# Enhex/RGK

Hardware: AMD Instinct MI355X
Metric: Mpaths/s, Sponza 1920x1080x256spp (path-tracing hot path) (higher is better)
Workload: dtype f32; 1 GPU; sponza-1080p 1920x1080x256spp depth 2 russian 0.74, strong scaling; geometry=proxy, triangles=64536, sampler=halton-cp, textures=handed over as u8; 0 of 0 float textures stored as bytes + value table, tiles=2040, parallelism=tiles round-robin over 1 GPU(s) + one RCCL reduce per round

## Files before the change

rgk_amd/csrc/rgk_host.cpp:

```cpp
#include <hip/hip_runtime.h>

#include <algorithm>
#include <array>
#include <atomic>
#include <cmath>
#include <cstdio>
#include <cstdlib>
#include <cstring>
#include <string>
#include <vector>

#include "../../include/rgk.h"
#include "device_types.h"
#include "rgk_commit.h"
#include "rgk_kernels.h"
#include "rgk_build.h"
#include "rgk_adapt.h"

namespace {

#define HIPCHK(x)                                                                                     \
    do {                                                                                              \
        hipError_t e_ = (x);                                                                          \
        if (e_ != hipSuccess)                                                                         \
// ... 23 lines not shown
            (void)hipDeviceSynchronize();
        }
        return 0;
    }
    int upload(const T* src, size_t count) {
        int rc = alloc(count);
        if (rc) return rc;
        if (count) {
            hipError_t e = hipMemcpy(p, src, count * sizeof(T), hipMemcpyHostToDevice);
            if (e != hipSuccess) return fail(RGK_ERR_DEVICE, "hipMemcpy H2D: %s", hipGetErrorString(e));
        }
        return 0;
    }
    void release() { if (p) (void)hipFree(p); p = nullptr; n = 0; }
};

}

struct RgkTuning {
    bool entry_points = true;
    bool entry_cap = true;
    bool light_entry = true;
    bool const_light = true;
    int sample_group = -1;
    size_t batch_paths = 0;
    double workspace_gb = 0;
    int beam = 1;
    bool debug_bvh = false, debug_util = false;
    bool time_post = false;
};

enum PostSlot : uint32_t { POST_AOV = 0, POST_DENOISE = 1, POST_DENOISE_VARIANCE = 2, POST_NOISE = 3, POST_FOLD = 4, POST_SLOTS = 5 };
constexpr uint32_t RGK_SCENE_MAGIC = 0x53474b52u;
struct rgk_scene {
    uint32_t magic = RGK_SCENE_MAGIC;
    int device = 0;
    RgkTuning tune;
    hipStream_t stream = nullptr;
    rgk_scene_info info{};
    DevScene dev{};
    RgkTraceCfg tcfg{32, 32, nullptr};
    DevBuf<int> ovf;
    DevBuf<QNode> nodes;
    DevBuf<TriIsect> tris;
    DevBuf<TriShade> tri_shade;
    DevBuf<DevMaterial> materials;
    DevBuf<float4> texels;
    DevBuf<uint32_t> texels8;
    DevBuf<float> luts;
    DevBuf<DevPointLight> pointlights;
    DevPointLight h_light0{};
    DevBuf<DevArealLight> areal;
    DevBuf<DevArealTri> areal_tris;
    DevBuf<float4> ltc;
    DevBuf<DevScene> self;
    DevBuf<uint32_t> generic;
    DevBuf<TexRef> texrefs;
    DevBuf<uint32_t> d_idx;
    DevBuf<float4> leaf_pb;
    std::vector<uint32_t> h_idx, h_tri_mat, h_areal_off, h_areal_tris;
    std::vector<rgk_material> h_mats;
    std::vector<float> h_normals;
    uint32_t n_vertices = 0, n_triangles = 0, n_refs = 0, n_nodes = 0;
    uint32_t n_textures = 0, n_materials = 0;
    DevBuf<DevHaltonDim> hdims;
    DevBuf<uint16_t> hperm;
    size_t batch = 0;
    DevBuf<float4> rayA[2], rayB[2], hit, thr, tot, shA, shB, shC, pixsum, light;
    DevBuf<float4> lstart, lv;
    DevBuf<uint32_t> hitlist;
    DevBuf<uint32_t> lvmask, connlist;
    DevBuf<float4> conn, jobs, rads;
    uint32_t batch_reverse = 0;
    DevBuf<float> htab;
    DevBuf<float2> nearfar;
    DevBuf<uint32_t> counters, pix_xy, pix_seed, tile_buf;
    DevBuf<int> entry;
    DevBuf<float> entry_cap;
    size_t entry_capped = 0;
    DevBuf<int> lentry;
    DevBuf<uint32_t> trange;
    DevBuf<float4> lbox;
    size_t lentry_done = 0;
    uint64_t entry_key = 0;
    size_t entry_n = 0;
    DevBuf<unsigned long long> stats;
    DevBuf<float> scratch_f;
    DevBuf<uint32_t> scratch_u;
    DevBuf<float4> dn_col[2], dn_guide;
    DevBuf<rgk_noise_tile> nz_tiles;
    DevBuf<uint32_t> fold_buf;
// ... 52 lines not shown
template <typename T>
int down(T* dst, const DevBuf<T>& b, size_t count) {
    if (hipMemcpy(dst, b.p, count * sizeof(T), hipMemcpyDeviceToHost) != hipSuccess) return fail(RGK_ERR_DEVICE, "hipMemcpy D2H failed");
    return 0;
}

int scene_event(rgk_scene* s, size_t i, hipEvent_t& e) {
    while (s->events.size() <= i) { hipEvent_t n; HIPCHK(hipEventCreate(&n)); s->events.push_back(n); }
    e = s->events[i];
    return 0;
}

int check_frame_size(uint32_t xres, uint32_t yres) {
    if (xres == 0 || yres == 0 || xres > 65535 || yres > 65535) return fail(RGK_ERR_INVALID, "resolution out of range");
    return RGK_OK;
}

int read_stats(const rgk_scene* s, unsigned long long (&h)[8]) { return down(h, s->stats, 8); }

RgkTuning read_tuning() {
    auto off = [](const char* name) { const char* e = std::getenv(name); return e && e[0] == '0'; };
    RgkTuning t;
    t.entry_points = !off("RGK_ENTRY_POINTS"); t.entry_cap = !off("RGK_ENTRY_CAP"); t.light_entry = !off("RGK_LIGHT_ENTRY");
    t.const_light = !off("RGK_CONST_LIGHT");
    if (const char* e = std::getenv("RGK_SAMPLE_GROUP")) t.sample_group = std::min(6, std::max(0, std::atoi(e)));
    if (const char* e = std::getenv("RGK_BATCH_PATHS")) t.batch_paths = std::max<size_t>(1024, strtoull(e, nullptr, 10));
    if (const char* e = std::getenv("RGK_WORKSPACE_GB")) t.workspace_gb = atof(e);
    if (const char* e = std::getenv("RGK_BEAM")) t.beam = std::min(2, std::max(0, std::atoi(e)));
    t.debug_bvh = std::getenv("RGK_DEBUG_BVH") != nullptr; t.debug_util = std::getenv("RGK_DEBUG_UTIL") != nullptr;
    return t;
}

void invalidate_frame_lists(rgk_scene* s) { s->entry_key = 0; s->entry_n = 0; s->entry_capped = 0; s->lentry_done = 0; }

void set_bounds(rgk_scene* s, const float mn[3], const float mx[3], float eps) {
    DevScene& ds = s->dev;
    ds.epsilon = eps;
    s->info.epsilon = eps;
    for (int a = 0; a < 3; a++) {
        ds.bb_min[a] = mn[a] - eps; ds.bb_max[a] = mx[a] + eps;
        s->info.bbox_min[a] = ds.bb_min[a]; s->info.bbox_max[a] = ds.bb_max[a];
    }
}

struct AccelInfo {
    uint32_t n_nodes = 0, n_refs = 0, max_depth = 0, max_stack = 0;
    bool on_device = false;
// ... 203 lines not shown
int rgk_scene_get_info(const rgk_scene* s, rgk_scene_info* out) {
    if (!s || !out) return fail(RGK_ERR_INVALID, "null argument");
    *out = s->info;
    return RGK_OK;
}

int rgk_scene_get_progress(const rgk_scene* s, rgk_progress* out) {
    if (!s || !out) return fail(RGK_ERR_INVALID, "null argument");
    out->stage = s->h_stage ? *(volatile const uint32_t*)s->h_stage : 0u; out->stages = s->prog_stages.load(); out->rounds = s->prog_rounds.load(); out->busy = s->prog_busy.load();
    out->round_pixels = s->prog_pixels.load(); out->round_paths = s->prog_paths.load();
    if (out->stage > out->stages) out->stage = out->stages;
    return RGK_OK;
}

int rgk_scene_set_tuning(rgk_scene* s, const char* key, double value) {
    if (!s || !key) return fail(RGK_ERR_INVALID, "null argument");
    if (s->prog_busy.load()) return fail(RGK_ERR_INVALID, "rgk_scene_set_tuning while a round is in flight on this scene");
    RgkTuning& t = s->tune;
    const std::string k(key);
    if (k == "entry_points") t.entry_points = value != 0;
    else if (k == "entry_cap") t.entry_cap = value != 0;
    else if (k == "light_entry") t.light_entry = value != 0;
    else if (k == "const_light") t.const_light = value != 0;
    else if (k == "sample_group") t.sample_group = value < 0 ? -1 : (int)std::min(6.0, value);
    else if (k == "batch_paths") t.batch_paths = value <= 0 ? 0 : std::max<size_t>(1024, (size_t)value);
    else if (k == "workspace_gb") t.workspace_gb = value <= 0 ? 0.0 : value;
    else if (k == "beam") t.beam = (int)std::min(2.0, std::max(0.0, value));
    else if (k == "time_post") { t.time_post = value != 0; return RGK_OK; }
    else return fail(RGK_ERR_INVALID, "unknown tuning key '%s'", key);
    invalidate_frame_lists(s);
    return RGK_OK;
}

int rgk_generate_task_list(uint32_t tile_size, uint32_t xres, uint32_t yres, float mid_x, float mid_y, uint32_t seedstart,
                           uint32_t seedcount_base, rgk_tile* tiles, uint32_t* n_tiles) {
    if (!n_tiles || tile_size == 0) return fail(RGK_ERR_INVALID, "bad argument");
    struct T { rgk_tile t; float d; };
    std::vector<T> v;
    for (uint32_t yp = 0; yp < yres; yp += tile_size)
        for (uint32_t xp = 0; xp < xres; xp += tile_size) {
            T t;
            t.t.x0 = xp; t.t.x1 = std::min(xres, xp + tile_size);
            t.t.y0 = yp; t.t.y1 = std::min(yres, yp + tile_size);
            t.t.seed = 0;
            float mx = (t.t.x0 + t.t.x1) / 2.0f, my = (t.t.y0 + t.t.y1) / 2.0f;
            float dx = mid_x - mx, dy = mid_y - my;
// ... 222 lines not shown
    if ((need_cap || need_light) && (rc = kl.run(RGK_K_OTHER, [&] { rgk_launch_group_trange(st, pp, s->hit.p, s->trange.p); }))) return rc;
    if (need_cap) {
        if ((rc = kl.run(RGK_K_OTHER, [&] { rgk_launch_entry_points(st, s->dev, cam, pp.xres, pp.yres, s->pix_xy.p, P, groups.first, groups.count(), s->trange.p, s->entry.p, s->entry_cap.p); })))
            return rc;
        s->entry_capped = end;
    }
    if (!light_entry) return 0;
    pp.lentry = s->lentry.p; pp.lbox = s->lbox.p;
    if (!need_light) return 0;
    if ((rc = kl.run(RGK_K_OTHER, [&] { rgk_launch_light_entry_points(st, s->dev, cam, pp, P, s->trange.p, s->lentry.p, s->lbox.p); }))) return rc;
    s->lentry_done = end;
    if (s->tune.debug_bvh) {
        const size_t g0 = groups.first, g1 = groups.last;
        std::vector<int> he((g1 - g0) * RGK_ENTRY_K);
        HIPCHK(hipStreamSynchronize(st));
        HIPCHK(hipMemcpy(he.data(), s->lentry.p + g0 * RGK_ENTRY_K, he.size() * sizeof(int), hipMemcpyDeviceToHost));
        size_t below = 0, total_e = 0;
        for (size_t g = 0; g < g1 - g0; g++) { if (he[g * RGK_ENTRY_K] != 0) below++; for (int k = 0; k < RGK_ENTRY_K; k++) total_e += he[g * RGK_ENTRY_K + k] != 0x7fffffff; }
        std::fprintf(stderr, "[rgk] light-side entry nodes: %zu of %zu pixel groups start below the root, %.2f entries per group\n", below, g1 - g0, (double)total_e / (double)(g1 - g0));
    }
    return 0;
}

int queue_pass(rgk_scene* s, KernelLog& kl, const DevCamera& cam, PassParams& pp, size_t P, bool light_entry, bool const_light, float* d_accum_rgb,
               uint32_t* d_accum_count, uint32_t stage) {
    hipStream_t st = s->stream;
    const RgkTraceCfg& tc = s->tcfg;
    const bool count_stats = kl.count_stats, cap_entries = s->entry.p != nullptr && s->tune.entry_cap;
    const bool track = pp.depth > 12;
    const uint32_t R = pp.reverse, n0 = pp.npix * pp.ns;
    pp.gshift = rgk_plan_gshift(s->tune.sample_group, RGK_SAMPLE_GROUP_DEFAULT, pp.ns);
    pp.beam = rgk_beam_wanted(s->tune.beam, cap_entries && (size_t)pp.j0 + pp.npix <= s->entry_capped) ? 1u : 0u;
    float4* const rayA[2] = {s->rayA[0].p, s->rayA[1].p};
    float4* const rayB[2] = {s->rayB[0].p, s->rayB[1].p};
    float4 *const hit = s->hit.p, *const thr = s->thr.p, *const tot = s->tot.p, *const shA = s->shA.p, *const shB = s->shB.p, *const shC = s->shC.p;
    uint32_t* const cn = s->counters.p;
    uint32_t* const cl = cn + RGK_CNT_TOTAL;
    int rc;
    if (R > 0) {
        if ((rc = kl.run(RGK_K_OTHER, [&] { rgk_launch_init_counters(st, cl, 0u); })) ||
            (rc = kl.run(RGK_K_LIGHT_SHADE, [&] { rgk_launch_raygen_light(st, s->dev, cam, pp, rayA[0], rayB[0], thr, cl); })))
            return rc;
        for (uint32_t k = 0; k < R; k++) {
            const int q = k & 1;
            if ((rc = kl.run(RGK_K_LIGHT_TRACE, [&] { rgk_launch_trace_closest(st, s->dev, tc, count_stats, rayA[q], rayB[q], nullptr, hit, {n0, cl + RGK_CNT_QUEUE + k, cl + RGK_CNT_FETCH_T + k}, s->stats.p); })) ||
                (rc = kl.run(RGK_K_LIGHT_SHADE, [&] { rgk_launch_list_hits(st, hit, cl + RGK_CNT_QUEUE + k, s->hitlist.p, cl + RGK_CNT_HITS + k, n0); })) ||
                (rc = kl.run(RGK_K_LIGHT_SHADE, [&] { rgk_launch_shade_light(st, s->dev, cam, pp, k, rayA[q], rayB[q], hit, thr, rayA[q ^ 1], rayB[q ^ 1], shA, shB, shC, cl, n0); })) ||
                (rc = kl.run(RGK_K_LIGHT_SPLAT, [&] { rgk_launch_trace_shadow(st, s->dev, tc, count_stats, shA, shB, shC, nullptr, nullptr, RGK_SHADOW_SPLAT, d_accum_rgb,
                                                                              {n0, cl + RGK_CNT_SHADOW + k, cl + RGK_CNT_FETCH_S + k}, s->stats.p); })))
                return rc;
        }
    }
    if ((rc = kl.run(RGK_K_OTHER, [&] { rgk_launch_init_counters(st, cn, n0); }))) return rc;
    uint32_t ub = n0;
    for (uint32_t b = 0; b < pp.depth && ub > 0; b++) {
        const int q = b & 1;
        const RgkWalk wq = {ub, cn + RGK_CNT_QUEUE + b, cn + RGK_CNT_FETCH_T + b}, ws = {ub, cn + RGK_CNT_SHADOW + b, cn + RGK_CNT_FETCH_S + b};
        if (b == 0)
            rc = kl.run(RGK_K_TRACE_CAMERA, [&] { rgk_launch_trace_camera(st, s->dev, cam, pp, tc, count_stats, hit, wq, s->stats.p); });
        else
            rc = kl.run(RGK_K_TRACE_CLOSEST, [&] { rgk_launch_trace_closest(st, s->dev, tc, count_stats, rayA[q], rayB[q], nullptr, hit, wq, s->stats.p); });
        if (rc || (b == 0 && (rc = queue_first_hit_lists(s, kl, cam, pp, (uint32_t)P, cap_entries, light_entry)))) return rc;
        if ((rc = kl.run(b == 0 ? RGK_K_SHADE_FIRST : RGK_K_SHADE, [&] { rgk_launch_shade(st, s->dev, cam, pp, b, rayA[q], rayB[q], hit, thr, tot, rayA[q ^ 1], rayB[q ^ 1], shA, shB, shC, cn, ub, R > 0, const_light); })) ||
            (R > 0 && (rc = kl.run(RGK_K_CONNECT, [&] { rgk_launch_connect(st, s->dev, pp, b, s->jobs.p, s->rads.p, cn, ub); }))))
            return rc;
        const bool first = b == 0 && light_entry, rec32 = const_light && rgk_const_light_records();
        rc = kl.run(first ? RGK_K_SHADOW_FIRST : RGK_K_SHADOW, [&] {
            if (rec32 && first) rgk_launch_trace_shadow_first_cl(st, s->dev, pp, tc, count_stats, shA, shB, tot, ws, s->stats.p);
            else if (rec32) rgk_launch_trace_shadow_cl(st, s->dev, tc, count_stats, shA, shB, tot, ws, s->stats.p);
            else if (first) rgk_launch_trace_shadow_first(st, s->dev, pp, tc, count_stats, shA, shB, shC, tot, ws, s->stats.p);
            else rgk_launch_trace_shadow(st, s->dev, tc, count_stats, shA, shB, shC, tot, nullptr, RGK_SHADOW_ADD, nullptr, ws, s->stats.p);
        });
        if (rc || (R > 0 && (rc = kl.run(RGK_K_SHADOW_JOBS, [&] { rgk_launch_trace_shadow_jobs(st, s->dev, pp, tc, count_stats, s->jobs.p, s->rads.p, tot, {ub, cn + RGK_CNT_CONN + b, cn + RGK_CNT_FETCH_J + b}, s->stats.p); }))))
            return rc;
        rgk_launch_stage_mark(st, s->h_stage, stage + b + 1);
        if (track && b >= 3 && (b & 1) && b + 1 < pp.depth && (rc = queue_len(s, cn + RGK_CNT_QUEUE + b + 1, ub))) return rc;
    }
    if ((rc = kl.run(RGK_K_RESOLVE, [&] { rgk_launch_resolve(st, pp, tot, s->pixsum.p, d_accum_rgb, d_accum_count); }))) return rc;
    rgk_launch_stage_mark(st, s->h_stage, stage + std::max(1u, pp.depth));
    HIPCHK(hipMemcpyAsync(s->h_counters, cn, 2 * RGK_CNT_TOTAL * sizeof(uint32_t), hipMemcpyDeviceToHost, st));
    return 0;
}
}

extern "C" {

// ... 17 lines not shown
    if ((rc = plan_passes(s, prm, P, R, plan))) return rc;

    DevCamera cam;
    make_camera(camera, cam);
    HIPCHK(hipMemsetAsync(s->stats.p, 0, 8 * sizeof(unsigned long long), s->stream));
    KernelLog kl(s, prm->flags);
    const uint32_t pass_stages = std::max(1u, prm->depth);
    {
        const uint32_t n_pix_passes = (uint32_t)((P + plan.npix_pass - 1) / plan.npix_pass), n_s_passes = (prm->multisample + plan.ns_pass - 1) / plan.ns_pass;
        *(volatile uint32_t*)s->h_stage = 0; s->prog_stages = n_pix_passes * n_s_passes * pass_stages;
        s->prog_pixels = P; s->prog_paths = (uint64_t)P * prm->multisample; s->prog_busy = 1;
    }
    struct Done { rgk_scene* s; ~Done() { *(volatile uint32_t*)s->h_stage = s->prog_stages.load(); s->prog_busy = 0; } } done_guard{s};
    PassParams pp{};
    pp.multisample = prm->multisample; pp.depth = prm->depth; pp.xres = prm->xres; pp.yres = prm->yres;
    pp.clamp = prm->clamp; pp.russian = prm->russian; pp.bumpmap_scale = prm->bumpmap_scale; pp.reverse = R;
    pp.lstart = s->lstart.p; pp.lv = s->lv.p; pp.hitlist = s->hitlist.p; pp.lvmask = s->lvmask.p; pp.conn = s->conn.p; pp.connlist = s->connlist.p;
    pp.batch = (uint32_t)s->batch;
    pp.pix_xy = s->pix_xy.p; pp.pix_seed = s->pix_seed.p; pp.light = s->light.p; pp.generic = s->generic.p;
    pp.entry = s->entry.p;
    pp.entry_cap = s->entry_cap.p;
    const bool light_entry = s->entry.p && s->tune.light_entry && s->dev.n_pointlights == 1 && s->dev.n_areal == 0;
    const bool const_light = s->info.const_light == 1 && s->tune.const_light && R == 0;
    if (light_entry) {
        const size_t groups = ((size_t)P + RGK_ENTRY_PIX - 1) / RGK_ENTRY_PIX + 1;
        if ((rc = s->lentry.alloc(groups * RGK_ENTRY_K)) || (rc = s->trange.alloc(groups * 2)) || (rc = s->lbox.alloc(groups * 2))) return rc;
    }
    if ((rc = s->htab.alloc((size_t)192 * prm->multisample))) return rc;
    if ((rc = kl.run(RGK_K_OTHER, [&] { rgk_launch_build_halton_table(s->stream, s->dev, prm->multisample, s->htab.p); }))) return rc;
    pp.htab = s->htab.p;

    rgk_counters tot{};
    uint32_t stage = 0;
    for (size_t j0 = 0; j0 < P; j0 += plan.npix_pass) {
        pp.j0 = (uint32_t)j0;
        pp.npix = (uint32_t)std::min(plan.npix_pass, P - j0);
        for (uint32_t s0 = 0; s0 < prm->multisample; s0 += plan.ns_pass, stage += pass_stages) {
            pp.s0 = s0;
            pp.ns = std::min(plan.ns_pass, prm->multisample - s0);
            if ((rc = queue_pass(s, kl, cam, pp, P, light_entry, const_light, d_accum_rgb, d_accum_count, stage))) return rc;
            HIPCHK(hipStreamSynchronize(s->stream));
            add_pass_counters(s->h_counters, pp, light_entry, tot);
        }
    }
    HIPCHK(hipGetLastError());
    s->prog_rounds++;
    if (counters) {
        tot.paths = (uint64_t)P * prm->multisample;
        if (kl.count_stats) {
            unsigned long long h[8];
            if ((rc = read_stats(s, h))) return rc;
            tot.node_visits = h[0]; tot.tri_tests = h[1]; tot.shadow_node_visits = h[2]; tot.shadow_tri_tests = h[3];
        }
        if ((rc = kl.fold(tot))) return rc;
        *counters = tot;
    }
    return RGK_OK;
}

int rgk_render_round(rgk_scene* s, const rgk_camera* camera, const rgk_params* prm, const rgk_tile* tiles, uint32_t n_tiles,
                     float* accum_rgb, uint32_t* accum_count, rgk_counters* counters) {
    if (!s || !prm || !accum_rgb || !accum_count) return fail(RGK_ERR_INVALID, "null argument");
    HIPCHK(hipSetDevice(s->device));
// ... 388 lines not shown
```

rgk_amd/csrc/rgk_kernels.h:

```cpp
#pragma once
#include <hip/hip_runtime.h>
#include "device_types.h"
#include "rgk_plan.h"

#ifndef RGK_SHADE_WAVES
#define RGK_SHADE_WAVES 4
#endif
#define RGK_MAX_DEPTH 62
#define RGK_LV_FLOAT4 6

#define RGK_CNT_QUEUE 0
#define RGK_CNT_SHADOW 64
#define RGK_CNT_FETCH_T 128
#define RGK_CNT_FETCH_S 192
#define RGK_CNT_GENERIC 256
#define RGK_CNT_HITS 320
#define RGK_CNT_SRAYS 384
#define RGK_CNT_CONN 448
#define RGK_CNT_FETCH_J 512
#define RGK_CNT_TOTAL 576

#define RGK_SHADOW_ADD 0
#define RGK_SHADOW_SPLAT 2

#ifndef RGK_ENTRY_K
#define RGK_ENTRY_K 6
#endif
struct PassParams {
    uint32_t j0, npix, s0, ns;
// ... 37 lines not shown
void rgk_launch_init_counters(hipStream_t st, uint32_t* counters, uint32_t n0);
void rgk_launch_build_pixel_list(hipStream_t st, const rgk_tile* tiles, const uint32_t* tile_off, uint32_t n_tiles, uint32_t* pix_xy, uint32_t* pix_seed);
void rgk_launch_build_halton_table(hipStream_t st, const DevScene& sc, uint32_t S, float* htab);
struct RgkWalk { uint32_t bound; const uint32_t* count_ptr; uint32_t* fetch; };
void rgk_launch_trace_camera(hipStream_t st, const DevScene& sc, const DevCamera& cam, const PassParams& pp, const RgkTraceCfg& tc, bool count_stats, float4* hit,
                             const RgkWalk& w, unsigned long long* stats);
void rgk_launch_trace_closest(hipStream_t st, const DevScene& sc, const RgkTraceCfg& tc, bool count_stats, const float4* rayA, const float4* rayB,
                              const float2* nearfar, float4* hit, const RgkWalk& w, unsigned long long* stats);
void rgk_launch_trace_shadow(hipStream_t st, const DevScene& sc, const RgkTraceCfg& tc, bool count_stats, const float4* shA, const float4* shB,
                             const float4* shC, float4* tot, uint8_t* vis_out, int mode, float* splat_rgb, const RgkWalk& w, unsigned long long* stats);
void rgk_launch_trace_shadow_first(hipStream_t st, const DevScene& sc, const PassParams& pp, const RgkTraceCfg& tc, bool count_stats, const float4* shA, const float4* shB,
                                   const float4* shC, float4* tot, const RgkWalk& w, unsigned long long* stats);
void rgk_launch_raygen_light(hipStream_t st, const DevScene& sc, const DevCamera& cam, const PassParams& pp, float4* rayA, float4* rayB,
                             float4* thr, uint32_t* counters);
void rgk_launch_shade_light(hipStream_t st, const DevScene& sc, const DevCamera& cam, const PassParams& pp, uint32_t k, const float4* rayA,
                            const float4* rayB, const float4* hit, float4* thr, float4* nextA, float4* nextB, float4* shA, float4* shB,
                            float4* shC, uint32_t* counters, uint32_t bound);
void rgk_launch_list_hits(hipStream_t st, const float4* hit, const uint32_t* count_ptr, uint32_t* list, uint32_t* list_count, uint32_t bound);
void rgk_launch_connect(hipStream_t st, const DevScene& sc, const PassParams& pp, uint32_t bounce, float4* jobs, float4* rads, uint32_t* counters, uint32_t bound);
void rgk_launch_trace_shadow_jobs(hipStream_t st, const DevScene& sc, const PassParams& pp, const RgkTraceCfg& tc, bool count_stats, const float4* jobs, const float4* rads,
                                  float4* tot, const RgkWalk& w, unsigned long long* stats);
void rgk_launch_shade(hipStream_t st, const DevScene& sc, const DevCamera& cam, const PassParams& pp, uint32_t bounce, const float4* rayA,
                      const float4* rayB, const float4* hit, float4* thr, float4* tot, float4* nextA, float4* nextB, float4* shA,
                      float4* shB, float4* shC, uint32_t* counters, uint32_t bound, bool bdpt = false, bool const_light = false);
bool rgk_const_light_records();
void rgk_launch_trace_shadow_cl(hipStream_t st, const DevScene& sc, const RgkTraceCfg& tc, bool count_stats, const float4* shA, const float4* shB,
                                float4* tot, const RgkWalk& w, unsigned long long* stats);
void rgk_launch_trace_shadow_first_cl(hipStream_t st, const DevScene& sc, const PassParams& pp, const RgkTraceCfg& tc, bool count_stats, const float4* shA, const float4* shB,
                                      float4* tot, const RgkWalk& w, unsigned long long* stats);
void rgk_launch_resolve(hipStream_t st, const PassParams& pp, const float4* tot, float4* pixsum, float* accum_rgb, uint32_t* accum_count);
void rgk_launch_pack_rays(hipStream_t st, uint32_t n, const float* rays, const int32_t* ignore, float4* rayA, float4* rayB, float2* nearfar);
void rgk_launch_pack_visibility(hipStream_t st, const DevScene& sc, uint32_t n, const float* a, const float* b, float4* shA, float4* shB,
                                float4* shC);
void rgk_launch_unpack_hits(hipStream_t st, uint32_t n, const float4* hit, rgk_hit* out);
void rgk_launch_sampler_eval(hipStream_t st, const DevScene& sc, uint32_t n, const uint32_t* seed, const uint32_t* index,
                             const uint32_t* dim, int is2d, float* out);

void rgk_launch_bxdf_value(hipStream_t st, const DevScene& sc, uint32_t n, uint32_t route, const uint32_t* mat, const float* Vi, const float* Vr, const float* uv, float* out);
void rgk_launch_bxdf_sample(hipStream_t st, const DevScene& sc, uint32_t n, uint32_t route, const uint32_t* mat, const float* Vi, const float* uv, const float* u,
                            float* out_dir, float* out_w, uint8_t* leak);
void rgk_launch_texture_sample(hipStream_t st, const DevScene& sc, uint32_t n, const TexRef* refs, const int32_t* tex, const float* uv, float* rgb, float* sr, float* sb);
void rgk_launch_libm_eval(hipStream_t st, int fn, uint32_t n, const float* a, const float* b, float* out);

void rgk_launch_aov_raygen(hipStream_t st, const DevCamera& cam, uint32_t xres, uint32_t yres, const uint32_t* pix_xy, uint32_t n, float4* rayA, float4* rayB);
void rgk_launch_aov_gather(hipStream_t st, const DevScene& sc, float bumpmap_scale, uint32_t xres, const uint32_t* pix_xy, uint32_t n, const float4* rayA,
                           const float4* rayB, const float4* hit, float* albedo, float* normal, float* depth, int32_t* tri);
void rgk_launch_dn_prepare(hipStream_t st, size_t P, const float* accum_rgb, const uint32_t* accum_count, const float* half_rgb, const uint32_t* half_count,
// ... 11 lines not shown
```

rgk_amd/csrc/rgk_kernels.hip:

```cpp
#include <hip/hip_runtime.h>
#include <cstdlib>
#include <type_traits>
#include "rgk_device.h"
#include "rgk_kernels.h"

#include "rgk_trace.h"

#ifndef RGK_SKIP_DEAD_NEE
#define RGK_SKIP_DEAD_NEE 1
#endif
#ifndef RGK_CL_REC32
#define RGK_CL_REC32 1
#endif



template <bool GENERIC, bool FIRST, bool BDPT = false, bool CL = false>
__global__ __launch_bounds__((FIRST ? RGK_SHADE_BLOCK : RGK_SHADE_BLOCK_LATER), RGK_SHADE_WAVES) void k_shade(const DevScene sc, const DevCamera cam, const PassParams pp, const uint32_t bounce,
                                                            const float4* __restrict__ rayA, const float4* __restrict__ rayB,
                                                            const float4* __restrict__ hit, float4* __restrict__ thr, float4* __restrict__ tot,
                                                            float4* __restrict__ nextA, float4* __restrict__ nextB, float4* __restrict__ shA,
                                                            float4* __restrict__ shB, float4* __restrict__ shC, uint32_t* __restrict__ counters) {
    const uint32_t count = counters[(GENERIC ? RGK_CNT_GENERIC : RGK_CNT_QUEUE) + bounce];
    const int lane = threadIdx.x & 63;
    const float eps = sc.epsilon;
    const SamplerTab tb = {pp.htab, pp.multisample};
    constexpr uint32_t BLK = FIRST ? RGK_SHADE_BLOCK : RGK_SHADE_BLOCK_LATER;
    __shared__ uint32_t s_cnt[4][BLK / 64];
    __shared__ uint32_t s_base[4];
    lut_lds_fill(sc);
    for (uint32_t base = blockIdx.x * BLK; base < count; base += gridDim.x * BLK) {
        const bool valid = base + threadIdx.x < count;
        const uint32_t i = !valid ? 0u : (GENERIC ? pp.generic[base + threadIdx.x] : base + threadIdx.x);
        bool cont = false, shadow = false, defer = false, conn = false;
        float4 nA = make_float4(0, 0, 0, 0), nB = nA, sA = nA, sB = nA, sC = nA;
        if (valid) {
            const float4 h = hit[i];
            uint32_t slot;
            f3 o, d;
            if (FIRST) { slot = i; camera_ray_of_slot(cam, pp, slot, o, d); }
            else {
                const float4 a = rayA[i], b = rayB[i];
                slot = __float_as_uint(b.w);
                o = mk3(a.x, a.y, a.z); d = mk3(a.w, b.x, b.y);
            }
            const float4 st = FIRST ? make_float4(1.f, 1.f, 1.f, __uint_as_float(1u << 16)) : thr[slot];
            const float4 li_slot = (FIRST || CL) ? make_float4(0.f, 0.f, 0.f, 0.f) : pp.light[slot];
            f3 tot0 = mk3(0.f, 0.f, 0.f);
            float4 li_keep = make_float4(0.f, 0.f, 0.f, 0.f);
            f3 cum = mk3(st.x, st.y, st.z);
            uint32_t bits = __float_as_uint(st.w);
            uint32_t n = (bits & 0xffffu) + 1u;
            uint32_t c1 = bits >> 16;
            const int tri = __float_as_int(h.w);
            uint32_t srel, j; slot_decode(pp, slot, j, srel);
            const uint32_t seed = pp.pix_seed[pp.j0 + j];
            const uint32_t s = pp.s0 + srel;
            const uint32_t base2d = (cam.lens_size != 0.0f) ? 2u : 1u;
            const f3 Vr = -d;
            if (tri < 0) {
                f3 sky = skybox(sc, Vr);
                f3 add = cum * sky;
                if (FIRST && !GENERIC) tot0 = mk3(0.f + add.x, 0.f + add.y, 0.f + add.z);
                else {
                    float4 t = tot[slot];
                    t.x = t.x + add.x; t.y = t.y + add.y; t.z = t.z + add.z;
                    tot[slot] = t;
                }
            } else {
// ... 18 lines not shown
                    faceN = norm3(faceN);
                    const float4 g3 = gld_f4(sc.tri_shade, tsr + 48u), g4 = gld_f4(sc.tri_shade, tsr + 64u), g5 = gld_f4(sc.tri_shade, tsr + 80u);
                    float2 uv = make_float2(0.f, 0.f);
                    if (sc.has_texcoords) {
                        uv.x = ia * g0.w + ib * g2.w + ic * g4.w;
                        uv.y = ia * g1.w + ib * g3.w + ic * g5.w;
                    }
                    const bool bumped = tex_kind(mat.t_bump) != RGK_TEXREF_NONE;
                    f3 lightN = faceN;
                    if (bumped) {
                        float right, bottom;
                        tex_slopes(sc, mat.t_bump, uv, right, bottom);
                        f3 tangent = ia * mk3(g3.x, g3.y, g3.z) + ib * mk3(g4.x, g4.y, g4.z) + ic * mk3(g5.x, g5.y, g5.z);
                        if (!(tangent.x * tangent.x + tangent.y * tangent.y + tangent.z * tangent.z < 0.001f)) {
                            tangent = norm3(tangent);
                            f3 bitangent = norm3(cross3(faceN, tangent));
                            f3 tangent2 = cross3(bitangent, faceN);
                            lightN = norm3(faceN + (tangent2 * right + bitangent * bottom) * pp.bumpmap_scale);
                            if (lightN.x != lightN.x) lightN = faceN;
                        }
                    }
                    const quatf g2l = rotation_between(lightN, mk3(0.f, 0.f, 1.f));
                    const f3 VrL = qrot(g2l, Vr);
                    const bool last = !(n < pp.depth);
                    const bool no_russian = (mat.flags & RGK_MAT_NO_RUSSIAN) != 0;
                    const bool ends = last;
                    float4 li;
                    if (CL) li = make_float4(sc.cl_pos[0], sc.cl_pos[1], sc.cl_pos[2], __uint_as_float(0u));
                    else if (FIRST) {
                        f3 lpos;
                        const uint32_t lcode = light_code(sc, sample2d_t(tb, seed, s, base2d + 2u), sample1d_t(tb, seed, s, 0u), sample2d_t(tb, seed, s, base2d), lpos);
                        li = make_float4(lpos.x, lpos.y, lpos.z, __uint_as_float(lcode));
                    } else li = li_slot;
                    bool nee_dead = false;
                    if (RGK_SKIP_DEAD_NEE && ends && !GENERIC) {
                        const DLight L0 = CL ? light_constant(sc) : light_from_code(sc, mk3(li.x, li.y, li.z), __float_as_uint(li.w));
                        if (L0.type < 0) nee_dead = true;
                        else {
                            const f3 df = pos - L0.pos;
                            nee_dead = dot3(df, df) > 0.f && (qrot(g2l, norm3(L0.pos - pos)).z <= 0.f || VrL.z <= 0.f);
                        }
                    }
                    MatPrep mp;
                    if (!nee_dead) mat_prepare(sc, mat, uv, VrL, !ends, mp);
                    else { mp.fast = true; mp.lobe = false; mp.diffc = mp.colorc = mk3(0.f, 0.f, 0.f); }
                    const f3 contribution = cum;
                    bool inside = false;
                    f3 dir = mk3(0.f, 0.f, 0.f);
                    uint32_t n_eff = n;
                    if (!ends) {
                        const quatf l2g = qinverse(g2l);
                        float2 u = sample2d_t(tb, seed, s, base2d + 3u + (n - 1u));
                        f3 dirL, weight; bool may_leak;
                        mat_sample<GENERIC>(sc, (int)mat_id, mat, mp, VrL, uv, u, dirL, weight, may_leak);
                        inside = dirL.z < 0;
                        dir = qrot(l2g, dirL);
                        if (!(dot3(dir, faceN) * dot3(Vr, faceN) > 0) && !may_leak) n_eff += 10000u;
                        const float rc = (!no_russian && pp.russian > 0.0f && n_eff > 1u) ? 1.0f / pp.russian : 1.0f;
                        cum = cum * rc;
                        cum = cum * weight;
                    }

                    {
                        li_keep = li;
                        const DLight L = CL ? light_constant(sc) : light_from_code(sc, mk3(li.x, li.y, li.z), __float_as_uint(li.w));
                        f3 e_front = mk3(0.f, 0.f, 0.f);
                        if (dot3(faceN, Vr) > 0) e_front = mk3(mat.emission[0], mat.emission[1], mat.emission[2]);
                        const bool has_e = (e_front.x != 0.f) || (e_front.y != 0.f) || (e_front.z != 0.f);
                        if (BDPT) conn = ((pp.lvmask[slot] & 0x7fu) != 0u) || has_e;
                        f3 B = mk3(0.f, 0.f, 0.f);
                        if (has_e && !conn) {
                            B = clamp3(mk3(0.f, 0.f, 0.f) + e_front, pp.clamp) * contribution;
                            if (FIRST && !GENERIC) tot0 = mk3(0.f + B.x, 0.f + B.y, 0.f + B.z);
// ... 20 lines not shown
                                if (rad.x != 0.f || rad.y != 0.f || rad.z != 0.f) {
                                    shadow = true;
                                    if (CL && RGK_CL_REC32) {
                                        sA = make_float4(sd.x, sd.y, sd.z, slen - eps * 20.0f);
                                        sB = make_float4(rad.x, rad.y, rad.z, __uint_as_float(slot));
                                    } else {
                                        sA = make_float4(L.pos.x, L.pos.y, L.pos.z, sd.x);
                                        sB = make_float4(sd.y, sd.z, slen - eps * 20.0f, __uint_as_float(slot));
                                        sC = make_float4(rad.x, rad.y, rad.z, 0.0f + eps * 20.0f);
                                    }
                                }
                            }
                        }
                        if (BDPT && conn) {
                            const size_t bs = pp.batch;
                            pp.conn[i] = make_float4(pos.x, pos.y, pos.z, __uint_as_float(slot));
                            pp.conn[bs + i] = make_float4(lightN.x, lightN.y, lightN.z, __uint_as_float(mat_id));
                            pp.conn[2 * bs + i] = make_float4(g2l.x, g2l.y, g2l.z, g2l.w);
                            pp.conn[3 * bs + i] = make_float4(VrL.x, VrL.y, VrL.z, uv.x);
                            pp.conn[4 * bs + i] = make_float4(contribution.x, contribution.y, contribution.z, uv.y);
                            pp.conn[5 * bs + i] = make_float4(out.x, out.y, out.z, __uint_as_float(has_e ? 1u : 0u));
                        }
                    }
                    bool go = !ends && !(max3c(cum) < 0.001f);
                    if (go && !no_russian && pp.russian >= 0.0f) {
                        float r = sample1d_t(tb, seed, s, c1);
                        c1++;
                        if (r > pp.russian) go = false;
                    }
                    if (go && n_eff > pp.depth) go = false;
                    if (go && !(n_eff < pp.depth)) go = false;
                    if (go) {
                        const float sgn = inside ? -1.0f : 1.0f;
                        f3 no = pos + faceN * eps * 10.0f * sgn;
                        f3 nd = norm3(norm3(dir));
                        cont = true;
                        nA = make_float4(no.x, no.y, no.z, nd.x);
                        nB = make_float4(nd.y, nd.z, __int_as_float(tri), __uint_as_float(slot));
                        thr[slot] = make_float4(cum.x, cum.y, cum.z, __uint_as_float((n & 0xffffu) | (c1 << 16)));
                    }
                    if (FIRST && !CL && (go || conn)) pp.light[slot] = li_keep;
                }
                }
            }
            if (FIRST && !GENERIC) tot[slot] = make_float4(tot0.x, tot0.y, tot0.z, 0.f);
        }
        {
            const unsigned long long m = __ballot(cont), ms = __ballot(shadow), md = __ballot(defer), mc = BDPT ? __ballot(conn) : 0ull;
            const int w = threadIdx.x >> 6;
            if (lane == 0) { s_cnt[0][w] = __popcll(m); s_cnt[1][w] = __popcll(ms); s_cnt[2][w] = __popcll(md); if (BDPT) s_cnt[3][w] = __popcll(mc); }
            __syncthreads();
            if (threadIdx.x == 0) {
                uint32_t t0 = 0, t1 = 0, t2 = 0, t3 = 0;
                for (int k = 0; k < (int)(BLK / 64); k++) {
                    uint32_t a = s_cnt[0][k], b = s_cnt[1][k], c = s_cnt[2][k];
                    s_cnt[0][k] = t0; s_cnt[1][k] = t1; s_cnt[2][k] = t2;
                    t0 += a; t1 += b; t2 += c;
                    if (BDPT) { uint32_t e = s_cnt[3][k]; s_cnt[3][k] = t3; t3 += e; }
                }
                s_base[0] = t0 ? atomicAdd(&counters[RGK_CNT_QUEUE + bounce + 1], t0) : 0u;
                s_base[1] = t1 ? atomicAdd(&counters[RGK_CNT_SHADOW + bounce], t1) : 0u;
                s_base[2] = t2 ? atomicAdd(&counters[RGK_CNT_GENERIC + bounce], t2) : 0u;
                if (BDPT) s_base[3] = t3 ? atomicAdd(&counters[RGK_CNT_CONN + bounce], t3) : 0u;
            }
            __syncthreads();
            if (!GENERIC && defer) pp.generic[s_base[2] + s_cnt[2][w] + __popcll(md & ((1ull << lane) - 1ull))] = i;
            if (BDPT && conn) pp.connlist[s_base[3] + s_cnt[3][w] + __popcll(mc & ((1ull << lane) - 1ull))] = i;
            if (cont) {
                uint32_t p = s_base[0] + s_cnt[0][w] + __popcll(m & ((1ull << lane) - 1ull));
                nextA[p] = nA; nextB[p] = nB;
            }
            if (shadow) {
                uint32_t p = s_base[1] + s_cnt[1][w] + __popcll(ms & ((1ull << lane) - 1ull));
                shA[p] = sA; shB[p] = sB;
                if (!(CL && RGK_CL_REC32)) shC[p] = sC;
            }
            __syncthreads();
        }
    }
}

#include "rgk_bdpt.h"

__global__ __launch_bounds__(256) void k_resolve(const PassParams pp, const float4* __restrict__ tot, float4* __restrict__ pixsum,
                                                  float* __restrict__ accum_rgb, uint32_t* __restrict__ accum_count) {
    for (uint32_t j = blockIdx.x * blockDim.x + threadIdx.x; j < pp.npix; j += gridDim.x * blockDim.x) {
        float4 acc = (pp.s0 == 0) ? make_float4(0.f, 0.f, 0.f, 0.f) : pixsum[pp.j0 + j];
        for (uint32_t srel = 0; srel < pp.ns; srel++) {
            float4 t = tot[slot_of(pp, j, srel)];
            f3 v = clamp3(mk3(t.x, t.y, t.z), pp.clamp);
            if (v.x != v.x || v.x < 0.0f) v.x = 0.0f;
            if (v.y != v.y || v.y < 0.0f) v.y = 0.0f;
            if (v.z != v.z || v.z < 0.0f) v.z = 0.0f;
// ... 414 lines not shown
        const int grid = rgk_bounded_grid(rgk_trace_grid(tc.lds), rgk_beam_bound(w.bound), RGK_TRACE_BLOCK);
        RGK_TRACE_LAUNCH(k_trace_camera_beam, 256, 8, sc, cam, pp, hit, w.count_ptr, w.fetch, stats, tc.ovf)
        return;
    }
    RGK_TRACE_DISPATCH(k_trace_camera, w.bound, sc, cam, pp, hit, w.count_ptr, w.fetch, stats, tc.ovf)
}

void rgk_launch_trace_closest(hipStream_t st, const DevScene& sc, const RgkTraceCfg& tc, bool count_stats, const float4* rayA, const float4* rayB,
                              const float2* nearfar, float4* hit, const RgkWalk& w, unsigned long long* stats) {
    RGK_TRACE_DISPATCH(k_trace_closest, w.bound, sc, rayA, rayB, nearfar, hit, w.count_ptr, w.fetch, stats, tc.ovf)
}

void rgk_launch_trace_shadow(hipStream_t st, const DevScene& sc, const RgkTraceCfg& tc, bool count_stats, const float4* shA, const float4* shB,
                             const float4* shC, float4* tot, uint8_t* vis_out, int mode, float* splat_rgb, const RgkWalk& w, unsigned long long* stats) {
    RGK_TRACE_DISPATCH(k_trace_shadow, w.bound, sc, shA, shB, shC, tot, vis_out, mode, splat_rgb, w.count_ptr, w.fetch, stats, tc.ovf)
}

void rgk_launch_trace_shadow_first(hipStream_t st, const DevScene& sc, const PassParams& pp, const RgkTraceCfg& tc, bool count_stats, const float4* shA, const float4* shB,
                                   const float4* shC, float4* tot, const RgkWalk& w, unsigned long long* stats) {
    RGK_TRACE_DISPATCH(k_trace_shadow_first, w.bound, sc, pp, shA, shB, shC, tot, w.count_ptr, w.fetch, stats, tc.ovf)
}

bool rgk_const_light_records() { return RGK_CL_REC32 != 0; }
void rgk_launch_trace_shadow_cl(hipStream_t st, const DevScene& sc, const RgkTraceCfg& tc, bool count_stats, const float4* shA, const float4* shB,
                                float4* tot, const RgkWalk& w, unsigned long long* stats) {
    RGK_TRACE_DISPATCH(k_trace_shadow_cl, w.bound, sc, shA, shB, tot, w.count_ptr, w.fetch, stats, tc.ovf)
}
void rgk_launch_trace_shadow_first_cl(hipStream_t st, const DevScene& sc, const PassParams& pp, const RgkTraceCfg& tc, bool count_stats, const float4* shA, const float4* shB,
                                      float4* tot, const RgkWalk& w, unsigned long long* stats) {
    RGK_TRACE_DISPATCH(k_trace_shadow_first_cl, w.bound, sc, pp, shA, shB, tot, w.count_ptr, w.fetch, stats, tc.ovf)
}

void rgk_launch_shade(hipStream_t st, const DevScene& sc, const DevCamera& cam, const PassParams& pp, uint32_t bounce, const float4* rayA,
                      const float4* rayB, const float4* hit, float4* thr, float4* tot, float4* nextA, float4* nextB, float4* shA,
                      float4* shB, float4* shC, uint32_t* counters, uint32_t bound, bool bdpt, bool const_light) {
    const RgkGridPair g = rgk_shade_grids(bounce, bound);
    auto pair = [&](auto first, auto bd, auto cl) {
        constexpr bool FIRST = decltype(first)::value, BDPT = decltype(bd)::value, CL = decltype(cl)::value;
        k_shade<false, FIRST, BDPT, CL><<<g.fast, g.block, RGK_LDS_SHADE_BYTES, st>>>(sc, cam, pp, bounce, rayA, rayB, hit, thr, tot, nextA, nextB, shA, shB, shC, counters);
        k_shade<true, FIRST, BDPT, CL><<<g.generic, g.block, RGK_LDS_SHADE_BYTES, st>>>(sc, cam, pp, bounce, rayA, rayB, hit, thr, tot, nextA, nextB, shA, shB, shC, counters);
    };
    constexpr std::true_type T{}; constexpr std::false_type F{};
    switch ((bounce == 0 ? 4 : 0) | (bdpt ? 2 : (const_light ? 1 : 0))) {
    case 4 | 2: pair(T, T, F); break;
    case 2: pair(F, T, F); break;
    case 4 | 1: pair(T, F, T); break;
    case 1: pair(F, F, T); break;
    case 4: pair(T, F, F); break;
    default: pair(F, F, F); break;
    }
}

void rgk_launch_resolve(hipStream_t st, const PassParams& pp, const float4* tot, float4* pixsum, float* accum_rgb, uint32_t* accum_count) {
    const RgkResolvePlan r = rgk_resolve_plan(pp.npix, pp.gshift);
    if (pp.gshift == 0) k_resolve<<<r.grid, 256, 0, st>>>(pp, tot, pixsum, accum_rgb, accum_count);
    else k_resolve_tiled<<<r.grid, 64, r.lds, st>>>(pp, tot, pixsum, accum_rgb, accum_count, r.PT);
}

void rgk_launch_pack_rays(hipStream_t st, uint32_t n, const float* rays, const int32_t* ignore, float4* rayA, float4* rayB, float2* nearfar) {
    k_pack_rays<<<(n + 255) / 256, 256, 0, st>>>(n, rays, ignore, rayA, rayB, nearfar);
}
void rgk_launch_pack_visibility(hipStream_t st, const DevScene& sc, uint32_t n, const float* a, const float* b, float4* shA, float4* shB, float4* shC) {
    k_pack_visibility<<<(n + 255) / 256, 256, 0, st>>>(sc, n, a, b, shA, shB, shC);
}
void rgk_launch_unpack_hits(hipStream_t st, uint32_t n, const float4* hit, rgk_hit* out) { k_unpack_hits<<<(n + 255) / 256, 256, 0, st>>>(n, hit, out); }
void rgk_launch_sampler_eval(hipStream_t st, const DevScene& sc, uint32_t n, const uint32_t* seed, const uint32_t* index, const uint32_t* dim,
                             int is2d, float* out) {
    k_sampler_eval<<<(n + 255) / 256, 256, 0, st>>>(sc, n, seed, index, dim, is2d, out);
}

void rgk_launch_raygen_light(hipStream_t st, const DevScene& sc, const DevCamera& cam, const PassParams& pp, float4* rayA, float4* rayB,
                             float4* thr, uint32_t* counters) {
// ... 20 lines not shown
```

Before: 4782 Mpaths/s.

## Specialize shade kernel for final bounce and queue throughput with continuation rays

Adds LAST and CUMQ template variants of the shade kernel. The last-bounce variant drops continuation sampling, the continuation ballot and atomics, and the next-ray writes. The variant for the second-to-last bounce writes path throughput into a compacted queue indexed like the next rays, so the last bounce reads it contiguously instead of gathering thr[slot]. This removes dead work and scattered reads in the final bounce, at the cost of more kernel instantiations and an extra buffer (which reuses the light buffer when constant lighting is on).

```diff
diff --git a/rgk_amd/csrc/rgk_host.cpp b/rgk_amd/csrc/rgk_host.cpp
--- a/rgk_amd/csrc/rgk_host.cpp
+++ b/rgk_amd/csrc/rgk_host.cpp
@@ -69,6 +69,7 @@
     bool entry_cap = true;
     bool light_entry = true;
     bool const_light = true;
+    bool last_kernel = true;
     int sample_group = -1;
     size_t batch_paths = 0;
     double workspace_gb = 0;
@@ -114,6 +115,7 @@
     DevBuf<uint16_t> hperm;
     size_t batch = 0;
     DevBuf<float4> rayA[2], rayB[2], hit, thr, tot, shA, shB, shC, pixsum, light;
+    DevBuf<float4> cumq;
     DevBuf<float4> lstart, lv;
     DevBuf<uint32_t> hitlist;
     DevBuf<uint32_t> lvmask, connlist;
@@ -212,7 +214,7 @@
     auto off = [](const char* name) { const char* e = std::getenv(name); return e && e[0] == '0'; };
     RgkTuning t;
     t.entry_points = !off("RGK_ENTRY_POINTS"); t.entry_cap = !off("RGK_ENTRY_CAP"); t.light_entry = !off("RGK_LIGHT_ENTRY");
-    t.const_light = !off("RGK_CONST_LIGHT");
+    t.const_light = !off("RGK_CONST_LIGHT"); t.last_kernel = !off("RGK_LAST_KERNEL");
     if (const char* e = std::getenv("RGK_SAMPLE_GROUP")) t.sample_group = std::min(6, std::max(0, std::atoi(e)));
     if (const char* e = std::getenv("RGK_BATCH_PATHS")) t.batch_paths = std::max<size_t>(1024, strtoull(e, nullptr, 10));
     if (const char* e = std::getenv("RGK_WORKSPACE_GB")) t.workspace_gb = atof(e);
@@ -462,6 +464,7 @@
     else if (k == "entry_cap") t.entry_cap = value != 0;
     else if (k == "light_entry") t.light_entry = value != 0;
     else if (k == "const_light") t.const_light = value != 0;
+    else if (k == "last_kernel") t.last_kernel = value != 0;
     else if (k == "sample_group") t.sample_group = value < 0 ? -1 : (int)std::min(6.0, value);
     else if (k == "batch_paths") t.batch_paths = value <= 0 ? 0 : std::max<size_t>(1024, (size_t)value);
     else if (k == "workspace_gb") t.workspace_gb = value <= 0 ? 0.0 : value;
@@ -730,8 +733,17 @@
     return 0;
 }
 
-int queue_pass(rgk_scene* s, KernelLog& kl, const DevCamera& cam, PassParams& pp, size_t P, bool light_entry, bool const_light, float* d_accum_rgb,
-               uint32_t* d_accum_count, uint32_t stage) {
+int last_cum_queue(rgk_scene* s, uint32_t depth, bool last_kernel, bool const_light, float4*& cumq) {
+    cumq = nullptr;
+    if (!last_kernel || depth < 2 || !rgk_last_cum_queue()) return 0;
+    if (const_light) { cumq = s->light.p; return 0; }
+    if (int rc = s->cumq.alloc(s->batch)) return rc;
+    cumq = s->cumq.p;
+    return 0;
+}
+
+int queue_pass(rgk_scene* s, KernelLog& kl, const DevCamera& cam, PassParams& pp, size_t P, bool light_entry, bool const_light, bool last_kernel, float4* cumq,
+               float* d_accum_rgb, uint32_t* d_accum_count, uint32_t stage) {
     hipStream_t st = s->stream;
     const RgkTraceCfg& tc = s->tcfg;
     const bool count_stats = kl.count_stats, cap_entries = s->entry.p != nullptr && s->tune.entry_cap;
@@ -769,7 +781,7 @@
         else
             rc = kl.run(RGK_K_TRACE_CLOSEST, [&] { rgk_launch_trace_closest(st, s->dev, tc, count_stats, rayA[q], rayB[q], nullptr, hit, wq, s->stats.p); });
         if (rc || (b == 0 && (rc = queue_first_hit_lists(s, kl, cam, pp, (uint32_t)P, cap_entries, light_entry)))) return rc;
-        if ((rc = kl.run(b == 0 ? RGK_K_SHADE_FIRST : RGK_K_SHADE, [&] { rgk_launch_shade(st, s->dev, cam, pp, b, rayA[q], rayB[q], hit, thr, tot, rayA[q ^ 1], rayB[q ^ 1], shA, shB, shC, cn, ub, R > 0, const_light); })) ||
+        if ((rc = kl.run(b == 0 ? RGK_K_SHADE_FIRST : RGK_K_SHADE, [&] { rgk_launch_shade(st, s->dev, cam, pp, b, rayA[q], rayB[q], hit, thr, tot, rayA[q ^ 1], rayB[q ^ 1], shA, shB, shC, cn, ub, R > 0, const_light, last_kernel, cumq); })) ||
             (R > 0 && (rc = kl.run(RGK_K_CONNECT, [&] { rgk_launch_connect(st, s->dev, pp, b, s->jobs.p, s->rads.p, cn, ub); }))))
             return rc;
         const bool first = b == 0 && light_entry, rec32 = const_light && rgk_const_light_records();
@@ -833,6 +845,9 @@
     pp.entry_cap = s->entry_cap.p;
     const bool light_entry = s->entry.p && s->tune.light_entry && s->dev.n_pointlights == 1 && s->dev.n_areal == 0;
     const bool const_light = s->info.const_light == 1 && s->tune.const_light && R == 0;
+    const bool last_kernel = s->tune.last_kernel && R == 0;
+    float4* cumq = nullptr;
+    if ((rc = last_cum_queue(s, prm->depth, last_kernel, const_light, cumq))) return rc;
     if (light_entry) {
         const size_t groups = ((size_t)P + RGK_ENTRY_PIX - 1) / RGK_ENTRY_PIX + 1;
         if ((rc = s->lentry.alloc(groups * RGK_ENTRY_K)) || (rc = s->trange.alloc(groups * 2)) || (rc = s->lbox.alloc(groups * 2))) return rc;
@@ -849,7 +864,7 @@
         for (uint32_t s0 = 0; s0 < prm->multisample; s0 += plan.ns_pass, stage += pass_stages) {
             pp.s0 = s0;
             pp.ns = std::min(plan.ns_pass, prm->multisample - s0);
-            if ((rc = queue_pass(s, kl, cam, pp, P, light_entry, const_light, d_accum_rgb, d_accum_count, stage))) return rc;
+            if ((rc = queue_pass(s, kl, cam, pp, P, light_entry, const_light, last_kernel, cumq, d_accum_rgb, d_accum_count, stage))) return rc;
             HIPCHK(hipStreamSynchronize(s->stream));
             add_pass_counters(s->h_counters, pp, light_entry, tot);
         }
diff --git a/rgk_amd/csrc/rgk_kernels.h b/rgk_amd/csrc/rgk_kernels.h
--- a/rgk_amd/csrc/rgk_kernels.h
+++ b/rgk_amd/csrc/rgk_kernels.h
@@ -5,6 +5,9 @@
 
 #ifndef RGK_SHADE_WAVES
 #define RGK_SHADE_WAVES 4
+#endif
+#ifndef RGK_SHADE_WAVES_LAST
+#define RGK_SHADE_WAVES_LAST 4
 #endif
 #define RGK_MAX_DEPTH 62
 #define RGK_LV_FLOAT4 6
@@ -88,7 +91,9 @@
                                   float4* tot, const RgkWalk& w, unsigned long long* stats);
 void rgk_launch_shade(hipStream_t st, const DevScene& sc, const DevCamera& cam, const PassParams& pp, uint32_t bounce, const float4* rayA,
                       const float4* rayB, const float4* hit, float4* thr, float4* tot, float4* nextA, float4* nextB, float4* shA,
-                      float4* shB, float4* shC, uint32_t* counters, uint32_t bound, bool bdpt = false, bool const_light = false);
+                      float4* shB, float4* shC, uint32_t* counters, uint32_t bound, bool bdpt = false, bool const_light = false,
+                      bool last_kernel = false, float4* cumq = nullptr);
+bool rgk_last_cum_queue();
 bool rgk_const_light_records();
 void rgk_launch_trace_shadow_cl(hipStream_t st, const DevScene& sc, const RgkTraceCfg& tc, bool count_stats, const float4* shA, const float4* shB,
                                 float4* tot, const RgkWalk& w, unsigned long long* stats);
diff --git a/rgk_amd/csrc/rgk_kernels.hip b/rgk_amd/csrc/rgk_kernels.hip
--- a/rgk_amd/csrc/rgk_kernels.hip
+++ b/rgk_amd/csrc/rgk_kernels.hip
@@ -9,18 +9,22 @@
 #ifndef RGK_SKIP_DEAD_NEE
 #define RGK_SKIP_DEAD_NEE 1
 #endif
+#ifndef RGK_LAST_CUMQ
+#define RGK_LAST_CUMQ 1
+#endif
 #ifndef RGK_CL_REC32
 #define RGK_CL_REC32 1
 #endif
 
 
 
-template <bool GENERIC, bool FIRST, bool BDPT = false, bool CL = false>
-__global__ __launch_bounds__((FIRST ? RGK_SHADE_BLOCK : RGK_SHADE_BLOCK_LATER), RGK_SHADE_WAVES) void k_shade(const DevScene sc, const DevCamera cam, const PassParams pp, const uint32_t bounce,
+template <bool GENERIC, bool FIRST, bool BDPT = false, bool CL = false, bool LAST = false, bool CUMQ = false>
+__global__ __launch_bounds__((FIRST ? RGK_SHADE_BLOCK : RGK_SHADE_BLOCK_LATER), (LAST ? RGK_SHADE_WAVES_LAST : RGK_SHADE_WAVES)) void k_shade(const DevScene sc, const DevCamera cam, const PassParams pp, const uint32_t bounce,
                                                             const float4* __restrict__ rayA, const float4* __restrict__ rayB,
                                                             const float4* __restrict__ hit, float4* __restrict__ thr, float4* __restrict__ tot,
-                                                            float4* __restrict__ nextA, float4* __restrict__ nextB, float4* __restrict__ shA,
+                                                            float4* __restrict__ nextA, float4* __restrict__ nextB, float4* __restrict__ cumq, float4* __restrict__ shA,
                                                             float4* __restrict__ shB, float4* __restrict__ shC, uint32_t* __restrict__ counters) {
+    static_assert(!(BDPT && (LAST || CUMQ)) && !(LAST && CUMQ), "bidirectional rounds keep the general kernel; a last vertex queues nothing");
     const uint32_t count = counters[(GENERIC ? RGK_CNT_GENERIC : RGK_CNT_QUEUE) + bounce];
     const int lane = threadIdx.x & 63;
     const float eps = sc.epsilon;
@@ -33,7 +37,7 @@
         const bool valid = base + threadIdx.x < count;
         const uint32_t i = !valid ? 0u : (GENERIC ? pp.generic[base + threadIdx.x] : base + threadIdx.x);
         bool cont = false, shadow = false, defer = false, conn = false;
-        float4 nA = make_float4(0, 0, 0, 0), nB = nA, sA = nA, sB = nA, sC = nA;
+        float4 nA = make_float4(0, 0, 0, 0), nB = nA, nC = nA, sA = nA, sB = nA, sC = nA;
         if (valid) {
             const float4 h = hit[i];
             uint32_t slot;
@@ -44,7 +48,7 @@
                 slot = __float_as_uint(b.w);
                 o = mk3(a.x, a.y, a.z); d = mk3(a.w, b.x, b.y);
             }
-            const float4 st = FIRST ? make_float4(1.f, 1.f, 1.f, __uint_as_float(1u << 16)) : thr[slot];
+            const float4 st = FIRST ? make_float4(1.f, 1.f, 1.f, __uint_as_float(1u << 16)) : ((LAST && RGK_LAST_CUMQ) ? cumq[i] : thr[slot]);
             const float4 li_slot = (FIRST || CL) ? make_float4(0.f, 0.f, 0.f, 0.f) : pp.light[slot];
             f3 tot0 = mk3(0.f, 0.f, 0.f);
             float4 li_keep = make_float4(0.f, 0.f, 0.f, 0.f);
@@ -109,7 +113,7 @@
                     }
                     const quatf g2l = rotation_between(lightN, mk3(0.f, 0.f, 1.f));
                     const f3 VrL = qrot(g2l, Vr);
-                    const bool last = !(n < pp.depth);
+                    const bool last = LAST || !(n < pp.depth);
                     const bool no_russian = (mat.flags & RGK_MAT_NO_RUSSIAN) != 0;
                     const bool ends = last;
                     float4 li;
@@ -129,13 +133,13 @@
                         }
                     }
                     MatPrep mp;
-                    if (!nee_dead) mat_prepare(sc, mat, uv, VrL, !ends, mp);
+                    if (!nee_dead) mat_prepare(sc, mat, uv, VrL, LAST ? false : !ends, mp);
                     else { mp.fast = true; mp.lobe = false; mp.diffc = mp.colorc = mk3(0.f, 0.f, 0.f); }
                     const f3 contribution = cum;
                     bool inside = false;
                     f3 dir = mk3(0.f, 0.f, 0.f);
                     uint32_t n_eff = n;
-                    if (!ends) {
+                    if (!LAST && !ends) {
                         const quatf l2g = qinverse(g2l);
                         float2 u = sample2d_t(tb, seed, s, base2d + 3u + (n - 1u));
                         f3 dirL, weight; bool may_leak;
@@ -202,7 +206,7 @@
                             pp.conn[5 * bs + i] = make_float4(out.x, out.y, out.z, __uint_as_float(has_e ? 1u : 0u));
                         }
                     }
-                    bool go = !ends && !(max3c(cum) < 0.001f);
+                    bool go = !LAST && !ends && !(max3c(cum) < 0.001f);
                     if (go && !no_russian && pp.russian >= 0.0f) {
                         float r = sample1d_t(tb, seed, s, c1);
                         c1++;
@@ -217,7 +221,8 @@
                         cont = true;
                         nA = make_float4(no.x, no.y, no.z, nd.x);
                         nB = make_float4(nd.y, nd.z, __int_as_float(tri), __uint_as_float(slot));
-                        thr[slot] = make_float4(cum.x, cum.y, cum.z, __uint_as_float((n & 0xffffu) | (c1 << 16)));
+                        if (CUMQ) nC = make_float4(cum.x, cum.y, cum.z, 0.f);
+                        else thr[slot] = make_float4(cum.x, cum.y, cum.z, __uint_as_float((n & 0xffffu) | (c1 << 16)));
                     }
                     if (FIRST && !CL && (go || conn)) pp.light[slot] = li_keep;
                 }
@@ -226,19 +231,20 @@
             if (FIRST && !GENERIC) tot[slot] = make_float4(tot0.x, tot0.y, tot0.z, 0.f);
         }
         {
-            const unsigned long long m = __ballot(cont), ms = __ballot(shadow), md = __ballot(defer), mc = BDPT ? __ballot(conn) : 0ull;
+            const unsigned long long m = LAST ? 0ull : __ballot(cont), ms = __ballot(shadow), md = __ballot(defer), mc = BDPT ? __ballot(conn) : 0ull;
             const int w = threadIdx.x >> 6;
-            if (lane == 0) { s_cnt[0][w] = __popcll(m); s_cnt[1][w] = __popcll(ms); s_cnt[2][w] = __popcll(md); if (BDPT) s_cnt[3][w] = __popcll(mc); }
+            if (lane == 0) { if (!LAST) s_cnt[0][w] = __popcll(m); s_cnt[1][w] = __popcll(ms); s_cnt[2][w] = __popcll(md); if (BDPT) s_cnt[3][w] = __popcll(mc); }
             __syncthreads();
             if (threadIdx.x == 0) {
                 uint32_t t0 = 0, t1 = 0, t2 = 0, t3 = 0;
                 for (int k = 0; k < (int)(BLK / 64); k++) {
-                    uint32_t a = s_cnt[0][k], b = s_cnt[1][k], c = s_cnt[2][k];
-                    s_cnt[0][k] = t0; s_cnt[1][k] = t1; s_cnt[2][k] = t2;
-                    t0 += a; t1 += b; t2 += c;
+                    uint32_t b = s_cnt[1][k], c = s_cnt[2][k];
+                    s_cnt[1][k] = t1; s_cnt[2][k] = t2;
+                    t1 += b; t2 += c;
+                    if (!LAST) { uint32_t a = s_cnt[0][k]; s_cnt[0][k] = t0; t0 += a; }
                     if (BDPT) { uint32_t e = s_cnt[3][k]; s_cnt[3][k] = t3; t3 += e; }
                 }
-                s_base[0] = t0 ? atomicAdd(&counters[RGK_CNT_QUEUE + bounce + 1], t0) : 0u;
+                if (!LAST) s_base[0] = t0 ? atomicAdd(&counters[RGK_CNT_QUEUE + bounce + 1], t0) : 0u;
                 s_base[1] = t1 ? atomicAdd(&counters[RGK_CNT_SHADOW + bounce], t1) : 0u;
                 s_base[2] = t2 ? atomicAdd(&counters[RGK_CNT_GENERIC + bounce], t2) : 0u;
                 if (BDPT) s_base[3] = t3 ? atomicAdd(&counters[RGK_CNT_CONN + bounce], t3) : 0u;
@@ -246,9 +252,10 @@
             __syncthreads();
             if (!GENERIC && defer) pp.generic[s_base[2] + s_cnt[2][w] + __popcll(md & ((1ull << lane) - 1ull))] = i;
             if (BDPT && conn) pp.connlist[s_base[3] + s_cnt[3][w] + __popcll(mc & ((1ull << lane) - 1ull))] = i;
-            if (cont) {
+            if (!LAST && cont) {
                 uint32_t p = s_base[0] + s_cnt[0][w] + __popcll(m & ((1ull << lane) - 1ull));
                 nextA[p] = nA; nextB[p] = nB;
+                if (CUMQ) cumq[p] = nC;
             }
             if (shadow) {
                 uint32_t p = s_base[1] + s_cnt[1][w] + __popcll(ms & ((1ull << lane) - 1ull));
@@ -709,6 +716,7 @@
 }
 
 bool rgk_const_light_records() { return RGK_CL_REC32 != 0; }
+bool rgk_last_cum_queue() { return RGK_LAST_CUMQ != 0; }
 void rgk_launch_trace_shadow_cl(hipStream_t st, const DevScene& sc, const RgkTraceCfg& tc, bool count_stats, const float4* shA, const float4* shB,
                                 float4* tot, const RgkWalk& w, unsigned long long* stats) {
     RGK_TRACE_DISPATCH(k_trace_shadow_cl, w.bound, sc, shA, shB, tot, w.count_ptr, w.fetch, stats, tc.ovf)
@@ -720,21 +728,27 @@
 
 void rgk_launch_shade(hipStream_t st, const DevScene& sc, const DevCamera& cam, const PassParams& pp, uint32_t bounce, const float4* rayA,
                       const float4* rayB, const float4* hit, float4* thr, float4* tot, float4* nextA, float4* nextB, float4* shA,
-                      float4* shB, float4* shC, uint32_t* counters, uint32_t bound, bool bdpt, bool const_light) {
+                      float4* shB, float4* shC, uint32_t* counters, uint32_t bound, bool bdpt, bool const_light, bool last_kernel, float4* cumq) {
     const RgkGridPair g = rgk_shade_grids(bounce, bound);
-    auto pair = [&](auto first, auto bd, auto cl) {
-        constexpr bool FIRST = decltype(first)::value, BDPT = decltype(bd)::value, CL = decltype(cl)::value;
-        k_shade<false, FIRST, BDPT, CL><<<g.fast, g.block, RGK_LDS_SHADE_BYTES, st>>>(sc, cam, pp, bounce, rayA, rayB, hit, thr, tot, nextA, nextB, shA, shB, shC, counters);
-        k_shade<true, FIRST, BDPT, CL><<<g.generic, g.block, RGK_LDS_SHADE_BYTES, st>>>(sc, cam, pp, bounce, rayA, rayB, hit, thr, tot, nextA, nextB, shA, shB, shC, counters);
+    auto pair = [&](auto first, auto bd, auto cl, auto la, auto cq) {
+        constexpr bool FIRST = decltype(first)::value, BDPT = decltype(bd)::value, CL = decltype(cl)::value, LAST = decltype(la)::value, CUMQ = decltype(cq)::value;
+        k_shade<false, FIRST, BDPT, CL, LAST, CUMQ><<<g.fast, g.block, RGK_LDS_SHADE_BYTES, st>>>(sc, cam, pp, bounce, rayA, rayB, hit, thr, tot, nextA, nextB, cumq, shA, shB, shC, counters);
+        k_shade<true, FIRST, BDPT, CL, LAST, CUMQ><<<g.generic, g.block, RGK_LDS_SHADE_BYTES, st>>>(sc, cam, pp, bounce, rayA, rayB, hit, thr, tot, nextA, nextB, cumq, shA, shB, shC, counters);
+    };
+    auto uni = [&](auto first, auto cl) {
+        constexpr std::true_type T{}; constexpr std::false_type F{};
+        if (last_kernel && bounce + 1 >= pp.depth) pair(first, F, cl, T, F);
+        else if (last_kernel && RGK_LAST_CUMQ && bounce + 2 == pp.depth) pair(first, F, cl, F, T);
+        else pair(first, F, cl, F, F);
     };
     constexpr std::true_type T{}; constexpr std::false_type F{};
     switch ((bounce == 0 ? 4 : 0) | (bdpt ? 2 : (const_light ? 1 : 0))) {
-    case 4 | 2: pair(T, T, F); break;
-    case 2: pair(F, T, F); break;
-    case 4 | 1: pair(T, F, T); break;
-    case 1: pair(F, F, T); break;
-    case 4: pair(T, F, F); break;
-    default: pair(F, F, F); break;
+    case 4 | 2: pair(T, T, F, F, F); break;
+    case 2: pair(F, T, F, F, F); break;
+    case 4 | 1: uni(T, T); break;
+    case 1: uni(F, T); break;
+    case 4: uni(T, F); break;
+    default: uni(F, F); break;
     }
 }
 
```

New measurement: 4790 Mpaths/s (median of 6 runs). About the same (+0.2%).
